# johannesschaeufele/CPUPathTrace

Measured on AMD Instinct MI355X. Metric: Msamples/s (all bounces), higher is better.
Workload: dtype f32

## Files before the change

### cpupathtrace_amd/csrc/pt_api.cpp

```cpp
#include "../../include/pt_hip.h"

#include <hip/hip_runtime.h>

#include <algorithm>
#include <chrono>
#include <cmath>
#include <cstdio>
#include <cstdlib>
#include <cstring>
#include <memory>
#include <mutex>
#include <string>
#include <thread>
#include <vector>

#include "pt_build.h"
#include "pt_bvh.h"
#include "pt_kernels.h"
#include "pt_post.h"

namespace {

thread_local std::string g_last_error;

// ... 102 lines not shown
struct pt_scene {
    int device = 0;
    hipStream_t stream = nullptr;
    int cu_count = 256;

    ptb::Tree tree;
    uint64_t n_nodes = 0;
    uint32_t depth = 0;
    bool device_built = false;
    float build_ms[4] = {0, 0, 0, 0};
    std::vector<uint32_t> tri_obj;
    std::vector<uint32_t> sph_obj;
    uint32_t n_objects = 0;
    uint32_t n_emissive = 0;
    std::vector<int32_t> emissive_obj;
    std::vector<float> emissive_cdf;

    DevBuf<F4> recs, pairs, tris, tri_shade, spheres, materials, lights, emis;
    DevBuf<uint2> sph_meta;
    DevBuf<float> emis_cdf;
    PtDevScene dev{};

    DevBuf<PtDevCounters> counters;
    DevBuf<F4> image;
    DevBuf<int4> tiles;
    DevBuf<uint32_t> tile_offset;
    DevBuf<float> batch_rays;

    std::mutex render_mutex;

    PtPathConfig path_cfg{};
    int path_blocks_per_cu = 0;
    uint32_t path_slots = 0, path_waves = 0, path_cap = 0;
    DevBuf<uint32_t> sl_stream, sl_nee_mask, pull_counter, tile_left;
    DevBuf<int4> sl_rect, st_rect;
    DevBuf<int32_t> sl_cursor, sl_path_length;
    DevBuf<uint64_t> sl_rng, st_rng;
    DevBuf<F4> sl_ray_o, sl_ray_d, sl_spectrum, sl_out, sl_nee, lq_ray_o, lq_ray_d;
    DevBuf<double> sl_divisor, sl_bounce_pd;
    DevBuf<PtEstimator> sl_est;
    DevBuf<PtCandidate> sl_cand;
    DevBuf<uint2> path_spill, closest_out;
    DevBuf<uint32_t> walk_save;
    DevBuf<PtPathArgs> path_args;
    PtPathArgs host_path_args{};
    DevBuf<unsigned long long> path_wave_counters;
    uint32_t *host_tiles_done = nullptr;
    unsigned long long *host_streams_done = nullptr;
    uint64_t streams_expected = 0;
    DevBuf<uint32_t> sl_cost, stream_cost, place;
    bool debug_collect_costs = false;
    std::vector<uint32_t> debug_place;
    uint32_t debug_place_waves = 0, debug_place_slots = 0;

    ~pt_scene() {
        if(host_tiles_done != nullptr) {
            (void)hipHostFree(host_tiles_done);
        }
        if(host_streams_done != nullptr) {
            (void)hipHostFree(host_streams_done);
        }
        if(stream != nullptr) {
            (void)hipStreamDestroy(stream);
        }
    }
};

namespace {

int device_count_quiet() {
    int n = 0;
    if(hipGetDeviceCount(&n) != hipSuccess) {
// ... 143 lines not shown
    if(slots_per_wave % first_lanes != 0) {
        if(slots_per_wave >= 64U) {
            slots_per_wave = (slots_per_wave + first_lanes - 1U) / first_lanes * first_lanes;
        }
        else {
            first_lanes = 1;
        }
    }
    cfg.first_lanes = static_cast<int>(first_lanes);
    int burst_default = 24;
    if(cfg.in_lds) {
        burst_default = slots_per_wave > 64U ? 12 : 24;
    }
    else if(slots_per_wave >= 64U) {
        burst_default = s->depth <= 12U ? 12 : (s->depth <= 18U ? 16 : 24);
    }
    cfg.burst_steps = std::min(std::max(env_int("PT_BURST", burst_default), 1), 64);
    int leaf_default = cfg.in_lds ? (slots_per_wave >= 64U ? 16 : 8) : static_cast<int>(std::min<uint32_t>(std::max<uint32_t>(slots_per_wave / 8U, 2U), 8U));
    if(!cfg.in_lds && slots_per_wave >= 64U && s->depth <= 24U) {
        leaf_default = 12;
    }
    cfg.leaf_min = std::min(std::max(env_int("PT_LEAF_MIN", leaf_default), 1), 64);
    const uint32_t rows = (slots_per_wave + 63U) / 64U;
    const uint32_t total = waves * rows * 64U;
    const uint32_t rays_per_slot = 1U + s->dev.n_lights + s->dev.n_object_samples;
    uint32_t cap = rows * 64U * rays_per_slot;
    const int ring_log = env_int("PT_RING_LOG_RAYS", 0);
    if(ring_log > 0) {
        cap = std::max<uint32_t>(cap, static_cast<uint32_t>(ring_log));
    }
    cfg.grid = static_cast<int>(grid);
    cfg.rows = static_cast<int>(rows);
    cfg.slots_per_wave = static_cast<int>(slots_per_wave);
    PT_HIP(s->sl_stream.ensure(total));
    PT_HIP(s->sl_rect.ensure(total));
    PT_HIP(s->sl_cursor.ensure(total));
    PT_HIP(s->sl_rng.ensure(total));
    PT_HIP(s->sl_ray_o.ensure(total));
    PT_HIP(s->sl_ray_d.ensure(total));
    PT_HIP(s->sl_spectrum.ensure(total));
    PT_HIP(s->sl_out.ensure(total));
    PT_HIP(s->sl_divisor.ensure(total));
    PT_HIP(s->sl_bounce_pd.ensure(total));
    PT_HIP(s->sl_path_length.ensure(total));
    PT_HIP(s->sl_nee.ensure(static_cast<size_t>(total) * std::max<uint32_t>(rays_per_slot - 1U, 1U)));
    PT_HIP(s->sl_nee_mask.ensure(total));
    PT_HIP(s->sl_cost.ensure(total));
    PT_HIP(s->sl_est.ensure(total));
    PT_HIP(s->sl_cand.ensure(static_cast<size_t>(total) * PT_MAX_CANDIDATES));
    PT_HIP(s->lq_ray_o.ensure(static_cast<size_t>(waves) * cap));
    PT_HIP(s->lq_ray_d.ensure(static_cast<size_t>(waves) * cap));
    if(ring_log > 0) {
        PT_HIP(hipMemsetAsync(s->lq_ray_d.ptr, 0xff, static_cast<size_t>(waves) * cap * 4 * sizeof(float), s->stream));
    }
    PT_HIP(s->path_spill.ensure(static_cast<size_t>(waves) * 64U * cfg.spill_depth));
    PT_HIP(s->path_wave_counters.ensure(static_cast<size_t>(waves) * 8U));
    PT_HIP(s->walk_save.ensure(static_cast<size_t>(waves) * 64U * PT_WALK_SAVE_WORDS));
    PT_HIP(s->pull_counter.ensure(64));
    PT_HIP(s->counters.ensure(1));
    cfg.spill = s->path_spill.ptr;
    cfg.walk_save = s->walk_save.ptr;
    cfg.wave_counters = s->path_wave_counters.ptr;
    s->path_slots = total;
    s->path_waves = waves;
    s->path_cap = cap;
    s->path_cfg.burst_steps = cfg.burst_steps;
    s->path_cfg.leaf_min = cfg.leaf_min;
    *out_cfg = cfg;
    return PT_OK;
}

int finish_path(pt_scene *s) {
    PT_HIP(hipStreamSynchronize(s->stream));
    if(s->host_streams_done != nullptr && s->streams_expected != 0) {
        const unsigned long long done = *static_cast<volatile unsigned long long *>(s->host_streams_done);
        const uint64_t expected = s->streams_expected;
        s->streams_expected = 0;
// ... 2 lines not shown
        }
    }
    return PT_OK;
}

int run_path(pt_scene *s, const PtDevCamera &cam, const PtDevOptions &opt, PtStreams T, float4 *d_image, pt_stats *stats, pt_progress_fn progress, void *progress_user,
             const PathPlan *plan = nullptr, bool want_costs = false) {
    PtPathConfig cfg;
    hipStream_t st = s->stream;
    PathPlan debug_plan;
    if(plan == nullptr && !s->debug_place.empty()) {
        PT_HIP(s->place.ensure(s->debug_place.size()));
        PT_HIP(hipMemcpyAsync(s->place.ptr, s->debug_place.data(), s->debug_place.size() * sizeof(uint32_t), hipMemcpyHostToDevice, st));
        PT_HIP(hipStreamSynchronize(st));
        debug_plan.waves = s->debug_place_waves;
        debug_plan.slots_per_wave = s->debug_place_slots;
        debug_plan.d_place = s->place.ptr;
        s->debug_place.clear();
        plan = &debug_plan;
    }
    int rc = ensure_path_workspace(s, T.n, &cfg, plan);
    if(rc != PT_OK) {
        return rc;
    }
    want_costs = want_costs || s->debug_collect_costs;
    T.place = plan != nullptr ? plan->d_place : nullptr;
    T.cost = nullptr;
    if(want_costs) {
        PT_HIP(s->stream_cost.ensure(std::max<uint32_t>(T.n, 1U)));
        T.cost = s->stream_cost.ptr;
    }
    PtSlots S{};
    S.total = s->path_slots;
    S.stream = s->sl_stream.ptr;
    S.rect = s->sl_rect.ptr;
    S.cursor = s->sl_cursor.ptr;
    S.rng = s->sl_rng.ptr;
    S.ray_o = reinterpret_cast<float4 *>(s->sl_ray_o.ptr);
    S.ray_d = reinterpret_cast<float4 *>(s->sl_ray_d.ptr);
    S.spectrum = reinterpret_cast<float4 *>(s->sl_spectrum.ptr);
    S.out = reinterpret_cast<float4 *>(s->sl_out.ptr);
    S.divisor = s->sl_divisor.ptr;
    S.bounce_pd = s->sl_bounce_pd.ptr;
    S.path_length = s->sl_path_length.ptr;
    S.nee = reinterpret_cast<float4 *>(s->sl_nee.ptr);
    S.nee_mask = s->sl_nee_mask.ptr;
    S.cost = s->sl_cost.ptr;
    S.est = s->sl_est.ptr;
    S.cand = s->sl_cand.ptr;
    PtLocalQueue Q{};
    Q.ray_o = reinterpret_cast<float4 *>(s->lq_ray_o.ptr);
    Q.ray_d = reinterpret_cast<float4 *>(s->lq_ray_d.ptr);
    Q.cap = s->path_cap;
    T.next = s->pull_counter.ptr;
    T.first_total = plan != nullptr ? T.n : s->path_waves * static_cast<uint32_t>(cfg.slots_per_wave);
    T.n_waves = s->path_waves;
    T.first_spread = env_int("PT_FIRST_SPREAD", 1) != 0 ? 1U : 0U;
    T.first_lanes = static_cast<uint32_t>(cfg.first_lanes);
    T.first_shift = static_cast<uint32_t>(std::max(env_int("PT_FIRST_SHIFT", 1), 0));
    {
        const uint32_t pieces = static_cast<uint32_t>(cfg.slots_per_wave) / T.first_lanes;
        const unsigned long long per_grid_row = static_cast<unsigned long long>(T.chunks_per_tile) * (64U / T.first_lanes) * T.tiles_per_row;
        if(env_int("PT_FIRST_SPREAD", 1) == 2 || per_grid_row == 0 || s->path_waves % per_grid_row != 0 || T.first_total > T.n || (T.tiles_per_row % pieces != 0 && pieces % T.tiles_per_row != 0)) {
            T.tiles_per_row = 0;
        }
    }
    T.tile_left = nullptr;
    T.tiles_done = nullptr;
    if(progress != nullptr && T.rect == nullptr && T.n_tiles > 0) {
        if(s->host_tiles_done == nullptr) {
            PT_HIP(hipHostMalloc(reinterpret_cast<void **>(&s->host_tiles_done), 64, hipHostMallocDefault));
        }
        *s->host_tiles_done = 0;
        T.tiles_done = s->host_tiles_done;
        T.tile_left = s->tile_left.ptr;
    }
    PT_HIP(hipMemsetAsync(s->counters.ptr, 0, sizeof(PtDevCounters), st));
// ... 1210 lines not shown
```

### cpupathtrace_amd/csrc/pt_kernels.h

```cpp
#ifndef PT_KERNELS_H
#define PT_KERNELS_H

#include <hip/hip_runtime.h>

#include "pt_types.h"

#define PT_F_DONE 1u
#define PT_F_IN_FLIGHT 2u
#define PT_F_HAS_EXT 4u
#define PT_F_COLLECTED 8u
#define PT_F_PIXEL 16u
#define PT_F_SAFE 64u
#define PT_F_OVERLAP 32u

#define PT_DEST_SHADOW 0x80000000u
#define PT_DEST_NULL 0xffffffffu


#define PT_LDS_TABLE_MAX 16
#define PT_LDS_TABLE_BYTES (PT_LDS_TABLE_MAX * (4 + 64 + 96 + 64))
#define PT_WALK_SAVE_WORDS 17
#define PT_MAX_ROWS 8
#define PT_F_STREAM 128u

struct PtSlots {
    uint32_t total;
    uint32_t *stream;
    int4 *rect;
    int32_t *cursor;
    uint64_t *rng;
    float4 *ray_o;
    float4 *ray_d;
    float4 *spectrum;
    float4 *out;
    double *divisor;
    double *bounce_pd;
    int32_t *path_length;
    float4 *nee;
    uint32_t *nee_mask;
    uint32_t *cost;
    PtEstimator *est;
    PtCandidate *cand;
};

struct PtStreams {
    uint32_t n;
    const int4 *rect;
    uint64_t *rng;
    const int4 *tiles;
    const uint32_t *tile_offset;
    uint32_t n_tiles;
    uint64_t base_seed;
    uint32_t first_total;
    uint32_t first_lanes;
    uint32_t first_shift;
    uint32_t n_waves, first_spread;
    uint32_t tiles_per_row, chunks_per_tile;
    uint32_t *next;
    uint32_t *tile_left;
    uint32_t *tiles_done;
    uint32_t *cost;
    const uint32_t *place;
};

struct PtLocalQueue {
    float4 *ray_o;
    float4 *ray_d;
    uint32_t cap;
};

// ... 54 lines not shown
```

### cpupathtrace_amd/csrc/pt_path.hip

```cpp
#include <type_traits>

#include "pt_device.h"
#include "pt_kernels.h"
#include "pt_shading.h"

using namespace ptd;

namespace {

typedef float f4v __attribute__((ext_vector_type(4)));
typedef float f2v __attribute__((ext_vector_type(2)));
typedef unsigned int u2v __attribute__((ext_vector_type(2)));
typedef const f4v __attribute__((address_space(3))) *lds_f4_cptr;
typedef const f4v __attribute__((address_space(1))) *glb_f4_cptr;
typedef u2v __attribute__((address_space(3))) *lds_u2_ptr;
typedef u2v __attribute__((address_space(1))) *glb_u2_ptr;
typedef unsigned int __attribute__((address_space(3))) *lds_u32_ptr;
typedef const PtPathArgs __attribute__((address_space(4))) *args_c4;

template<bool IN_LDS>
struct RecPtr {
    typedef glb_f4_cptr type;
};
template<>
// ... 73 lines not shown
#endif
    typedef typename RecPtr<IN_LDS>::type rec_ptr;
    rec_ptr recs;
    lds_u2_ptr stack_l;
    glb_u2_ptr my_spill;

    struct Rec {
        f4v r0, r1, r2, r3;
    };
    PT_D void fetch(uint32_t cur, Rec &R) const {
        rec_ptr p = recs + 4 * (size_t)(cur & PT_REF_INDEX);
        R.r0 = p[0];
        R.r1 = p[1];
        R.r2 = p[2];
        R.r3 = p[3];
    }
    static PT_D void whole(const Rec &R) {
        asm volatile("" ::"v"(R.r0), "v"(R.r1), "v"(R.r2), "v"(R.r3));
    }

    static PT_D unsigned long long node_lanes(uint32_t cur) { return __builtin_amdgcn_uicmp(cur, 0x40000000u, 36); }
    static PT_D unsigned long long slow_lanes(uint32_t cur) { return __builtin_amdgcn_uicmp(cur + 1u, 0x40000000u, 34); }

    PT_D void start(Walk &w, Rec &R, const RootBox &root, float4 ro, float4 rd) const {
        w.o = v3(ro.x, ro.y, ro.z);
        w.d = v3(rd.x, rd.y, rd.z);
        w.thr = ro.w;
        w.dest = __float_as_uint(rd.w);
        w.inv = slab_inverse(w.d);
        w.pack();
        w.best_ref = PT_REF_NONE;
        w.best_t = -1.0f;
        w.set_t_max(FLT_MAX);
        const u2v sentinel = {PT_REF_NONE, __float_as_uint(-1.0f)};
        stack_l[0] = sentinel;
        w.sp = 1;
        w.occluded = false;
        w.cur = PT_REF_NONE;
        if(root.ref != PT_REF_NONE) {
            const float t_root = slab_walk(ld3(root.lo), ld3(root.hi), w.o, w.inv);
            if(t_root >= 0.0f) {
                w.cur = root.ref;
                fetch(w.cur, R);
            }
        }
    }

    PT_D void node_step(Walk &w, Rec &R, unsigned long long node_mask, unsigned long long deep_mask) const {
        if(!__builtin_amdgcn_inverse_ballot_w64(node_mask)) {
            return;
        }
#ifdef PT_STEP_STAMPS
        asm volatile("s_waitcnt vmcnt(0)" ::: "memory");
#endif
        PT_STAMP(2);
        whole(R);
        const f4v q0 = R.r0, q1 = R.r1, q2 = R.r2;
        const uint32_t sp = w.sp;
        const u2v top = stack_l[((sp - 1u) & (uint32_t)(STACK_LDS - 1)) * 256u];
        const f2v a0 = ((f2v){q0.x, q0.y} - w.o_xy) * w.i_xy;
        const f2v a1 = ((f2v){q0.z, q0.w} - w.o_zx) * w.i_zx;
        const f2v a2 = ((f2v){q1.x, q1.y} - w.o_yz) * w.i_yz;
        const f2v a3 = ((f2v){q1.z, q1.w} - w.o_xy) * w.i_xy;
        const f2v a4 = ((f2v){q2.x, q2.y} - w.o_zx) * w.i_zx;
        const f2v a5 = ((f2v){q2.z, q2.w} - w.o_yz) * w.i_yz;
        const float l1 = a0.x, l2 = a1.y, l3 = a0.y, l4 = a2.x, l5 = a1.x, l6 = a2.y;
        const float r1 = a3.x, r2 = a4.y, r3 = a3.y, r4 = a5.x, r5 = a4.x, r6 = a5.y;
// ... 167 lines not shown
        if(T.tile_offset[mid] <= i) {
            lo = mid;
        }
        else {
            hi = mid;
        }
    }
    const int4 t = T.tiles[lo];
    const uint32_t k = i - T.tile_offset[lo];
    const int32_t x = t.x + (int32_t)(k % (uint32_t)t.z), y = t.y + (int32_t)(k / (uint32_t)t.z);
    rect = make_int4(x, y, 1, 1);
    const uint64_t seed = pixel_seed(T.base_seed, x, y);
    rng = seed ^ (~seed << 32);
    tile = lo;
}

struct EmisLds {
    const float __attribute__((address_space(3))) *cdf_l;
    lds_f4_cptr rec_l;
    lds_f4_cptr light_l;
    PT_D float cdf(int i) const { return cdf_l[i]; }
    PT_D float4 rec(int i, int k) const { return to_f4(rec_l[4 * i + k]); }
    PT_D V3 tri_normal_at(int i, uint32_t, V3 pos) const {
        uint32_t mat_unused;
        return tri_shade_normal(light_l + 6 * i, pos, mat_unused);
    }
};
struct ShadeTables {
    EmisLds emis;
    lds_f4_cptr materials_l;
    bool emis_in_lds, materials_in_lds;
};

template<bool WIDE>
PT_D void shade_row(const PtDevScene &sc, const PtDevCamera &cam, const PtDevOptions &opt, const PtSlots &S, const PtStreams &T, const PtLocalQueue &Q,
                    WaveCtx &ctx, uint32_t row, uint32_t ls_in, uint32_t lane, size_t slot_base, size_t queue_base, typename SlotWord<WIDE>::lds_ptr word_l, lds_u2_ptr hit_l,
                    float4 *__restrict__ image, PtDevCounters *counters, const ShadeTables &tb, uint32_t &n_samples, uint32_t &n_vertices) {
    const bool have_slot = ls_in != PT_NO_SLOT;
    const uint32_t ls = have_slot ? ls_in : 0u;
    const size_t p = slot_base + ls;
    const unsigned long long lt = (1ULL << lane) - 1ULL;
    const uint32_t n_light_samples = sc.n_lights + sc.n_object_samples;
    typedef SlotWord<WIDE> SW;
    const typename SW::T word = word_l[ls];
    uint32_t flags = SW::flags(word);
    const uint32_t vis_bits = SW::vis(word);
    bool ready = have_slot && !(flags & PT_F_DONE) && SW::pending(word) == 0;
    if(__ballot(ready) == 0ULL) {
        return;
    }

    {
        const bool want = ready && !(flags & PT_F_STREAM);
        const unsigned long long want_mask = __ballot(want);
        if(want_mask != 0ULL) {
            uint32_t base = T.n;
            uint32_t mine;
            if((ctx.first_rows >> row) & 1u) {
                ctx.first_rows &= ~(1u << row);
                base = ctx.first_base + row * 64u;
                mine = base + lane;
                if(T.place != nullptr) {
                    base = 0;
                    mine = T.place[ctx.first_base + ls];
                }
                else if(T.first_spread) {
                    const uint32_t g = T.first_lanes, q = row * (64u / g) + lane / g;
                    uint32_t chunk = q * T.n_waves + ctx.wave;
                    if(T.tiles_per_row != 0) {
                        const uint32_t per_tile = T.chunks_per_tile * (64u / g), pieces = (T.first_total / T.n_waves) / g;
                        const uint32_t tile = chunk / per_tile, sub = chunk % per_tile;
                        const uint32_t step = T.tiles_per_row >= pieces ? T.tiles_per_row / pieces : 1u;
                        const uint32_t tx = (tile % T.tiles_per_row + q * T.first_shift * step) % T.tiles_per_row, ty = tile / T.tiles_per_row;
                        chunk = (ty * T.tiles_per_row + tx) * per_tile + sub;
                    }
                    base = 0;
                    mine = chunk * g + lane % g;
                }
            }
            else {
                if(!ctx.pool_empty) {
                    if(lane == 0) {
                        base = T.first_total + atomicAdd(T.next, (uint32_t)__popcll(want_mask));
                    }
                    base = __builtin_amdgcn_readfirstlane(base);
                }
                mine = base + (uint32_t)__popcll(want_mask & lt);
                if(base >= T.n || base + (uint32_t)__popcll(want_mask) > T.n) {
                    ctx.pool_empty = true;
                }
            }
            const bool got = want && base < T.n && mine < T.n;
            if(got) {
                int4 rc;
                uint64_t r;
                uint32_t tile = 0;
                if(T.rect != nullptr) {
                    rc = T.rect[mine];
                    r = T.rng[mine];
                }
                else {
                    tile_stream(T, mine, rc, r, tile);
                }
                S.stream[p] = mine;
                S.rect[p] = rc;
                S.rng[p] = r;
                S.cursor[p] = 0;
                if(T.cost != nullptr) {
                    __hip_atomic_store(&S.cost[p], 0u, __ATOMIC_RELAXED, __HIP_MEMORY_SCOPE_AGENT);
                }
                flags = PT_F_STREAM;
            }
            else if(want) {
                flags = PT_F_DONE;
                ready = false;
                word_l[ls] = SW::make(PT_F_DONE, 0u, 0u, 0u);
            }
            ctx.n_dead += (uint32_t)__popcll(__ballot(want && !got));
        }
    }
    const bool alive = ready;
    uint32_t lane_samples = 0;

    uint64_t rng = 0;
    C4 out = c4(0, 0, 0, 0), spectrum = c4(1, 1, 1, 1);
    V3 ro = v3(0, 0, 0), rd = v3(0, 0, 1);
    float contribution_unweighted = 1.0f;
    double divisor = 1.0, bounce_pd = 1.0;
    int path_length = 0;
    bool shade_vertex = false;
    bool start_sample = false;
    float hit_t = -1.0f;
    uint32_t hit_ref = PT_REF_NONE;
    int4 rect = make_int4(0, 0, 0, 0);
    int32_t cursor = 0;
    bool stream_finished = false;

    if(alive) {
        rng = S.rng[p];
        rect = S.rect[p];
        cursor = S.cursor[p];
        if(flags & PT_F_IN_FLIGHT) {
            const float4 out4 = S.out[p];
            uint32_t mask = SW::waiting(word, S, p);
            const uint32_t lit = mask & vis_bits;
            float4 nee0 = make_float4(0, 0, 0, 0), nee1 = make_float4(0, 0, 0, 0);
            if(lit & 1u) {
                nee0 = S.nee[p];
            }
            if(lit & 2u) {
                nee1 = S.nee[S.total + p];
            }
            const float4 o4 = S.ray_o[p], d4 = S.ray_d[p], spectrum4 = S.spectrum[p];
            const double divisor_in = S.divisor[p], bounce_pd_in = S.bounce_pd[p];
            const int path_length_in = S.path_length[p];
            uint32_t warm = 0;
            if(flags & PT_F_HAS_EXT) {
                const u2v h = hit_l[ls];
                hit_t = __uint_as_float(h.x);
                hit_ref = h.y;
                if(!(hit_t < 0.0f) && !(hit_ref & PT_REF_SPHERE)) {
                    warm = *reinterpret_cast<const uint32_t *>(sc.tri_shade + 8 * (size_t)(hit_ref & PT_REF_INDEX));
                }
            }
            out = c4(out4);
            if(lit & 1u) {
                out = out + c4(nee0);
            }
            if(lit & 2u) {
                out = out + c4(nee1);
            }
            mask >>= 2;
            for(uint32_t j = 2; mask != 0; j++, mask >>= 1) {
                if((mask & 1u) && ((vis_bits >> j) & 1u)) {
                    out = out + c4(S.nee[(size_t)j * S.total + p]);
                }
            }
            asm volatile("" ::"v"(warm));
            if(flags & PT_F_OVERLAP) {
                PtEstimator e = S.est[p];
                out.a = 1.0f;
                (void)estimator_add(e, S.cand + p * PT_MAX_CANDIDATES, opt, out);
                e.pixel_sample++;
                lane_samples++;
                S.est[p] = e;
                flags &= ~(PT_F_OVERLAP | PT_F_COLLECTED | PT_F_SAFE);
                if(estimator_safe_to_overlap(e, opt)) {
                    flags |= PT_F_SAFE;
                }
                out = c4(0, 0, 0, 0);
            }
            bool finished = true;
            if((flags & PT_F_HAS_EXT) && !(hit_t < 0.0f)) {
                finished = false;
                shade_vertex = true;
            }
            if(finished) {
                PtEstimator e = S.est[p];
                PtCandidate *cand = S.cand + p * PT_MAX_CANDIDATES;
                bool accepted = false;
                if(flags & PT_F_COLLECTED) {
                    out.a = 1.0f;
                    accepted = estimator_add(e, cand, opt, out);
                }
                e.pixel_sample++;
                lane_samples++;
                if(accepted || e.pixel_sample >= opt.max_sample_count) {
                    const C4 value = estimator_finish(e, cand, opt, accepted);
                    const int32_t px = rect.x + cursor % rect.z, py = rect.y + cursor / rect.z;
                    image[(size_t)py * opt.image_width + px] = f4(value);
                    cursor++;
                    flags &= ~PT_F_PIXEL;
                }
                S.est[p] = e;
                flags &= ~(PT_F_IN_FLIGHT | PT_F_HAS_EXT | PT_F_COLLECTED | PT_F_SAFE);
                if((flags & PT_F_PIXEL) && estimator_safe_to_overlap(e, opt)) {
                    flags |= PT_F_SAFE;
                }
                start_sample = true;
            }
            else {
                ro = v3(o4.x, o4.y, o4.z);
                rd = v3(d4.x, d4.y, d4.z);
                contribution_unweighted = o4.w;
                spectrum = c4(spectrum4);
                divisor = divisor_in;
                bounce_pd = bounce_pd_in;
                path_length = path_length_in;
            }
        }
        else {
            start_sample = true;
        }
    }

    bool emit_ext = false;
    Ray ext;
    ext.o = v3(0, 0, 0);
    ext.d = v3(0, 0, 1);
    auto shoot_camera = [&](const int4 rc, int32_t cur) {
        const int32_t px = rc.x + cur % rc.z, py = rc.y + cur / rc.z;
        const float one_half = 1.0f / 2.0f;
        const float x_camera = 2 * (((float)px + one_half) / (float)opt.image_width - one_half);
        float y_camera = 2 * (((float)py + one_half) / (float)opt.image_height - one_half);
        y_camera = -y_camera;
        return camera_shoot(cam, x_camera, y_camera, opt.pixel_width, opt.pixel_height, rng);
    };
    if(start_sample) {
        bool have_pixel = false;
        while(cursor < rect.z * rect.w) {
            if(!(flags & PT_F_PIXEL)) {
                PtEstimator e;
                estimator_reset(e, opt);
                S.est[p] = e;
                flags = (flags | PT_F_PIXEL) & ~PT_F_SAFE;
                if(estimator_safe_to_overlap(e, opt)) {
                    flags |= PT_F_SAFE;
                }
                if(opt.max_sample_count <= 0) {
                    const int32_t px = rect.x + cursor % rect.z, py = rect.y + cursor / rect.z;
                    image[(size_t)py * opt.image_width + px] = make_float4(0.0f, 0.0f, 0.0f, 0.0f);
                    cursor++;
                    flags &= ~PT_F_PIXEL;
                    continue;
                }
            }
            have_pixel = true;
            break;
        }
        if(!have_pixel) {
            stream_finished = true;
            flags = 0;
        }
        else {
            ext = shoot_camera(rect, cursor);
            emit_ext = true;
            out = c4(0, 0, 0, 0);
            spectrum = c4(1, 1, 1, 1);
            contribution_unweighted = 1.0f;
            divisor = 1.0;
            bounce_pd = 1.0;
            path_length = 0;
            flags |= PT_F_IN_FLIGHT | PT_F_HAS_EXT;
        }
    }
    {
        const unsigned long long fin_mask = __ballot(stream_finished);
        if(fin_mask != 0ULL) {
            if(stream_finished) {
                const uint32_t si = S.stream[p];
                if(T.rng != nullptr) {
                    T.rng[si] = rng;
                }
                if(T.cost != nullptr) {
                    T.cost[si] = __hip_atomic_load(&S.cost[p], __ATOMIC_RELAXED, __HIP_MEMORY_SCOPE_AGENT);
                }
                if(T.tile_left != nullptr) {
                    int4 rc_unused;
                    uint64_t r_unused;
                    uint32_t tile = 0;
                    tile_stream(T, si, rc_unused, r_unused, tile);
                    if(atomicSub(&T.tile_left[tile], 1u) == 1u) {
                        __hip_atomic_fetch_add(T.tiles_done, 1u, __ATOMIC_RELAXED, __HIP_MEMORY_SCOPE_SYSTEM);
                    }
                }
            }
            if(lane == 0) {
                atomicAdd(&counters->streams_done, (unsigned long long)__popcll(fin_mask));
            }
        }
    }

    V3 pos = v3(0, 0, 0), n = v3(0, 1, 0);
    Material mat;
    mat.bsdf = 0;
    bool do_bounce = false;
    float bounce_probability = 1.0f;
    bool want_nee = false;
    bool safe_overlap = false;
    if(shade_vertex) {
        path_length++;
        flags |= PT_F_COLLECTED;
        pos = ro + rd * hit_t;
// ... 108 lines not shown
            }
        }
        const bool path_ends = !do_bounce || cancel_ext;
        if(path_ends && safe_overlap) {
            ext = shoot_camera(rect, cursor);
            spectrum = c4(1, 1, 1, 1);
            contribution_unweighted = 1.0f;
            divisor = 1.0;
            bounce_pd = 1.0;
            path_length = 0;
            flags |= PT_F_OVERLAP;
        }
        else if(path_ends && emit_ext) {
            Q.ray_d[ring(ext_pos)] = make_float4(0.0f, 0.0f, 0.0f, __uint_as_float(PT_DEST_NULL));
            emit_ext = false;
        }
        if(emit_ext) {
            flags |= PT_F_HAS_EXT;
        }
        else {
            flags &= ~PT_F_HAS_EXT;
        }
    }

    if(emit_ext) {
        const size_t at = ring(ext_pos);
        Q.ray_o[at] = make_float4(ext.o.x, ext.o.y, ext.o.z, 0.0f);
        Q.ray_d[at] = make_float4(ext.d.x, ext.d.y, ext.d.z, __uint_as_float(ls));
        n_rays++;
    }
    if(alive) {
        word_l[ls] = SW::make(flags, n_rays, vis_init, nee_out_mask);
        SW::keep_waiting(S, p, nee_out_mask);
        S.rng[p] = rng;
        S.cursor[p] = cursor;
        if(flags & PT_F_IN_FLIGHT) {
            S.ray_o[p] = make_float4(ext.o.x, ext.o.y, ext.o.z, contribution_unweighted);
            S.ray_d[p] = make_float4(ext.d.x, ext.d.y, ext.d.z, 0.0f);
            S.spectrum[p] = f4(spectrum);
            S.out[p] = f4(out);
            S.divisor[p] = divisor;
            S.bounce_pd[p] = bounce_pd;
            S.path_length[p] = path_length;
        }
    }
    n_samples += (uint32_t)__popcll(__ballot(lane_samples & 1u)) + 2u * (uint32_t)__popcll(__ballot((lane_samples & 2u) != 0u));
    n_vertices += (uint32_t)__popcll(__ballot(shade_vertex));
}


#define PT_PATH_STACK_LDS 8
#define PT_PATH_STACK_LDS_SMALL 4
#ifndef PT_COST_LDS_BYTES
#define PT_COST_LDS_BYTES 1024
#endif
#ifndef PT_PATH_WAVES
#define PT_PATH_WAVES 4
#endif

template<bool WIDE, bool IN_LDS, int STACK_LDS>
__global__ __launch_bounds__(256, PT_PATH_WAVES) void pt_path_kernel(const PtPathArgs *__restrict__ args) {
    typedef SlotWord<WIDE> SW;
    const args_c4 A4 = (args_c4)args;
    const PtPathArgs *A = (const PtPathArgs *)A4;
    const int rows = A->rows, slots_per_wave = A->slots_per_wave, refill_idle = A->refill_idle, min_ready = A->min_ready, burst_steps = A->burst_steps,
              leaf_min = A->leaf_min, ready_shift = A->ready_shift, pass_q_low = A->early_ready > 0 ? A->pass_q_low : 0, early_ready = A->early_ready;
    const unsigned long long lane_cap = A->debug_lanes >= 64 ? ~0ULL : ((1ULL << A->debug_lanes) - 1ULL);
    PtLocalQueue Q = A->Q;
    RootBox root;
    root.ref = A->sc.root_ref;
    for(int k = 0; k < 3; k++) {
        root.lo[k] = A->sc.root_lo[k];
        root.hi[k] = A->sc.root_hi[k];
    }
    extern __shared__ __align__(16) unsigned char lds_raw[];
    const int tid = threadIdx.x;
    const uint32_t lane = (uint32_t)tid & 63u;
    const uint32_t wave_in_block = __builtin_amdgcn_readfirstlane((uint32_t)tid >> 6);
    const uint32_t wave = blockIdx.x * 4u + wave_in_block;
    const uint32_t n_slots = (uint32_t)rows * 64u;
    unsigned char *at = lds_raw;
    lds_u2_ptr stack_l = (lds_u2_ptr)reinterpret_cast<uint2 *>(at) + tid;
    at += (size_t)STACK_LDS * 256 * sizeof(uint2);
    lds_u2_ptr hit_l = (lds_u2_ptr)reinterpret_cast<uint2 *>(at) + wave_in_block * n_slots;
    at += (size_t)4 * n_slots * sizeof(uint2);
    typename SW::lds_ptr word_l = (typename SW::lds_ptr)reinterpret_cast<typename SW::T *>(at) + wave_in_block * n_slots;
    at += (size_t)4 * n_slots * sizeof(typename SW::T);
    float *cdf_l = reinterpret_cast<float *>(at);
    at += (size_t)PT_LDS_TABLE_MAX * sizeof(float);
    float4 *emis_l = reinterpret_cast<float4 *>(at);
    at += (size_t)PT_LDS_TABLE_MAX * 4 * sizeof(float4);
    float4 *light_l = reinterpret_cast<float4 *>(at);
    at += (size_t)PT_LDS_TABLE_MAX * 6 * sizeof(float4);
    float4 *materials_l = reinterpret_cast<float4 *>(at);
    at += (size_t)PT_LDS_TABLE_MAX * 4 * sizeof(float4);
    uint32_t __attribute__((address_space(3))) *born_l = (uint32_t __attribute__((address_space(3))) *)reinterpret_cast<uint32_t *>(at) + tid;
    typedef unsigned char __attribute__((address_space(3))) *lds_u8_ptr;
    lds_u8_ptr list_l = (lds_u8_ptr)reinterpret_cast<unsigned char *>(at) + wave_in_block * 256u;
    at += (size_t)PT_COST_LDS_BYTES;
    float4 *lds_recs = reinterpret_cast<float4 *>(at);
    const bool cost_on = PT_COST_LDS_BYTES != 0 && A->T.cost != nullptr;
    uint32_t *const slot_cost = A->S.cost;

    ShadeTables tb;
    tb.emis.cdf_l = (const float __attribute__((address_space(3))) *)cdf_l;
    tb.emis.rec_l = (lds_f4_cptr)emis_l;
    tb.emis.light_l = (lds_f4_cptr)light_l;
    tb.materials_l = (lds_f4_cptr)materials_l;
    {
        const uint32_t n_emis = A->sc.n_emis, n_materials = A->sc.n_materials;
        tb.emis_in_lds = n_emis > 0 && n_emis <= PT_LDS_TABLE_MAX;
        tb.materials_in_lds = n_materials > 0 && n_materials <= PT_LDS_TABLE_MAX;
        if(tb.emis_in_lds) {
            const float4 *src_emis = A->sc.emis, *src_shade = A->sc.tri_shade;
            const float *src_cdf = A->sc.emis_cdf;
            for(uint32_t i = tid; i < n_emis; i += 256) {
                cdf_l[i] = src_cdf[i];
            }
            for(uint32_t i = tid; i < 4 * n_emis; i += 256) {
                emis_l[i] = src_emis[i];
            }
            for(uint32_t i = tid; i < 6 * n_emis; i += 256) {
                const uint32_t ref = __float_as_uint(src_emis[4 * (i / 6) + 2].y);
                light_l[i] = (ref & PT_REF_SPHERE) ? make_float4(0, 0, 0, 0) : src_shade[8 * (size_t)(ref & PT_REF_INDEX) + i % 6];
            }
        }
        if(tb.materials_in_lds) {
            const float4 *src_materials = A->sc.materials;
            for(uint32_t i = tid; i < 4 * n_materials; i += 256) {
                materials_l[i] = src_materials[i];
            }
        }
    }

    if(IN_LDS) {
        const uint32_t n_lds_quads = 4u * (A->sc.pair_base + A->sc.n_pairs);
        const float4 *src_recs = A->sc.recs;
        for(uint32_t i = tid; i < n_lds_quads; i += 256) {
            lds_recs[i] = src_recs[i];
        }
    }
    for(uint32_t i = lane; i < n_slots; i += 64) {
        word_l[i] = i < (uint32_t)slots_per_wave ? (typename SW::T)0 : SW::make(PT_F_DONE, 0u, 0u, 0u);
    }
    __syncthreads();

    Tracer<STACK_LDS, IN_LDS> tr;
    if(IN_LDS) {
        tr.recs = (typename RecPtr<IN_LDS>::type)(lds_f4_cptr)lds_recs;
    }
    else {
        tr.recs = (typename RecPtr<IN_LDS>::type)(glb_f4_cptr)A->sc.recs;
    }
    tr.stack_l = stack_l;
    tr.my_spill = (glb_u2_ptr)(A->spill + ((size_t)wave * 64 + lane) * A->spill_depth);

    const size_t slot_base = (size_t)wave * n_slots;
    const size_t queue_base = (size_t)wave * Q.cap;
    WaveCtx ctx;
    ctx.q_head = 0;
    ctx.q_count = 0;
    ctx.n_dead = n_slots - (uint32_t)slots_per_wave;
    ctx.pool_empty = false;
    ctx.first_rows = (1u << rows) - 1u;
    ctx.first_base = wave * (uint32_t)slots_per_wave;
    ctx.wave = wave;

    bool active = false;
    Walk w;
    w.o = v3(0, 0, 0);
    w.d = v3(0, 0, 1);
    w.inv = v3(0, 0, 0);
    w.pack();
    w.thr = 0.0f;
    w.dest = 0;
    w.best_t = 0.0f;
    w.best_ref = PT_REF_NONE;
    w.set_t_max(FLT_MAX);
    w.cur = PT_REF_NONE;
    w.sp = 0;
    w.occluded = false;
    typename Tracer<STACK_LDS, IN_LDS>::Rec rec;
    rec.r0 = rec.r1 = rec.r2 = rec.r3 = (f4v){0.0f, 0.0f, 0.0f, 0.0f};
    float4 win_o = make_float4(0, 0, 0, 0), win_d = make_float4(0, 0, 0, __uint_as_float(PT_DEST_NULL));
    uint32_t n_nodes = 0, n_leaves = 0, n_rays = 0, n_shadow = 0, n_samples = 0, n_vertices = 0;
    uint32_t w_steps = 0, w_passes = 0;
#ifdef PT_PATH_TIMING
    unsigned long long t_shade = 0, t_burst = 0;
    const unsigned long long t_begin = __builtin_amdgcn_s_memtime();
#endif

    bool want_pass = false;
    for(;;) {
        if(want_pass) {
            want_pass = false;
            w_passes++;
#ifdef PT_PATH_TIMING
            const unsigned long long t_pass = __builtin_amdgcn_s_memtime();
#endif
            size_t pass_offset = 0;
            asm volatile("" : "+s"(pass_offset));
            const PtPathArgs *P = (const PtPathArgs *)(args_c4)((const char __attribute__((address_space(4))) *)A4 + pass_offset);
            uint32_t *const walk_save = P->walk_save;
            const size_t save_stride = P->save_stride;
            {
                uint32_t *sv = walk_save + (size_t)wave * 64 + lane;
                const size_t st = save_stride;
                sv[0 * st] = __float_as_uint(w.o.x);
                sv[1 * st] = __float_as_uint(w.o.y);
                sv[2 * st] = __float_as_uint(w.o.z);
                sv[3 * st] = __float_as_uint(w.d.x);
                sv[4 * st] = __float_as_uint(w.d.y);
                sv[5 * st] = __float_as_uint(w.d.z);
                sv[6 * st] = __float_as_uint(w.thr);
                sv[7 * st] = w.dest;
                sv[8 * st] = __float_as_uint(w.best_t);
                sv[9 * st] = w.best_ref;
                sv[10 * st] = __float_as_uint(w.t_max);
                sv[11 * st] = w.cur;
                sv[12 * st] = w.sp | (w.occluded ? 0x80000000u : 0u);
                sv[13 * st] = n_nodes;
                sv[14 * st] = n_leaves;
                sv[15 * st] = n_rays;
                sv[16 * st] = n_shadow;
            }
            uint32_t n_listed = 0;
            bool compact = false;
            if(PT_COST_LDS_BYTES >= 1024 && !cost_on && P->compact_passes != 0 && rows > 1 && rows <= 4 && ctx.first_rows == 0u) {
                uint32_t rows_used = 0;
                for(uint32_t r = 0; r < (uint32_t)rows; r++) {
                    const typename SW::T word = word_l[r * 64 + lane];
                    const bool is_ready = !(SW::flags(word) & PT_F_DONE) && SW::pending(word) == 0;
                    const unsigned long long m = __ballot(is_ready);
                    if(is_ready) {
                        list_l[n_listed + (uint32_t)__popcll(m & ((1ULL << lane) - 1ULL))] = (unsigned char)(r * 64 + lane);
                    }
                    n_listed += (uint32_t)__popcll(m);
                    rows_used += m != 0ULL ? 1u : 0u;
                }
                compact = (n_listed + 63u) / 64u < rows_used;
                __builtin_amdgcn_fence(__ATOMIC_ACQ_REL, "workgroup");
            }
            const uint32_t n_chunks = compact ? (n_listed + 63u) / 64u : (uint32_t)rows;
#pragma unroll 1
            for(uint32_t k = 0; k < n_chunks; k++) {
                uint32_t ls = k * 64u + lane;
                if(compact) {
                    ls = ls < n_listed ? (uint32_t)list_l[ls] : PT_NO_SLOT;
                }
                shade_row<WIDE>(P->sc, P->cam, P->opt, P->S, P->T, P->Q, ctx, k, ls, lane, slot_base, queue_base, word_l, hit_l, P->image, P->counters, tb, n_samples, n_vertices);
            }
            __builtin_amdgcn_fence(__ATOMIC_ACQ_REL, "workgroup");
            __builtin_amdgcn_s_waitcnt(0);
            {
                asm volatile("" : "+s"(pass_offset));
                const PtPathArgs *R = (const PtPathArgs *)(args_c4)((const char __attribute__((address_space(4))) *)A4 + pass_offset);
                const uint32_t *sv = R->walk_save + (size_t)wave * 64 + lane;
                const size_t st = R->save_stride;
                w.o = v3(__uint_as_float(sv[0 * st]), __uint_as_float(sv[1 * st]), __uint_as_float(sv[2 * st]));
                w.d = v3(__uint_as_float(sv[3 * st]), __uint_as_float(sv[4 * st]), __uint_as_float(sv[5 * st]));
                w.inv = slab_inverse(w.d);
                w.pack();
                w.thr = __uint_as_float(sv[6 * st]);
                w.dest = sv[7 * st];
                w.best_t = __uint_as_float(sv[8 * st]);
                w.best_ref = sv[9 * st];
                w.set_t_max(__uint_as_float(sv[10 * st]));
                w.cur = sv[11 * st];
                const uint32_t packed = sv[12 * st];
                w.sp = packed & 0x7fffffffu;
                w.occluded = (packed >> 31) != 0;
                n_nodes = sv[13 * st];
                n_leaves = sv[14 * st];
                n_rays = sv[15 * st];
                n_shadow = sv[16 * st];
            }
#ifdef PT_PATH_TIMING
            t_shade += __builtin_amdgcn_s_memtime() - t_pass;
#endif
            win_o = make_float4(0, 0, 0, 0);
            win_d = make_float4(0, 0, 0, __uint_as_float(PT_DEST_NULL));
            if(lane < ctx.q_count) {
                uint32_t i = ctx.q_head + lane;
                i = i >= Q.cap ? i - Q.cap : i;
                win_o = Q.ray_o[queue_base + i];
                win_d = Q.ray_d[queue_base + i];
            }
            rec.r0 = rec.r1 = rec.r2 = rec.r3 = (f4v){0.0f, 0.0f, 0.0f, 0.0f};
                    if(active && w.cur < PT_REF_POPPING) {
                tr.fetch(w.cur, rec);
            }
        }

        bool finished = false;
        for(;;) {
            if(active && w.cur == PT_REF_NONE) {
                const uint32_t ls = w.dest & PT_DEST_SLOT_MASK;
                if(w.dest & PT_DEST_SHADOW) {
                    const uint32_t j = (w.dest >> PT_DEST_J_SHIFT) & SW::j_mask;
                    __hip_atomic_fetch_add(&word_l[ls], (typename SW::T)(w.occluded ? 0u : (1u << j)) - SW::one_ray(), __ATOMIC_RELAXED, __HIP_MEMORY_SCOPE_WORKGROUP);
                }
                else {
                    const u2v h = {__float_as_uint(w.best_ref == PT_REF_NONE ? -1.0f : w.best_t), w.best_ref};
                    hit_l[ls] = h;
                    __hip_atomic_fetch_add(&word_l[ls], (typename SW::T)0 - SW::one_ray(), __ATOMIC_RELAXED, __HIP_MEMORY_SCOPE_WORKGROUP);
                }
                if(cost_on) {
                    __hip_atomic_fetch_add(&slot_cost[slot_base + ls], w_steps - *born_l, __ATOMIC_RELAXED, __HIP_MEMORY_SCOPE_AGENT);
                }
                active = false;
            }

            const unsigned long long idle_mask = __ballot(!active) & lane_cap;
            const uint32_t n_idle = (uint32_t)__popcll(idle_mask);
            if(n_idle >= (uint32_t)refill_idle) {
                if(ctx.q_count <= (uint32_t)pass_q_low && ctx.n_dead < n_slots) {
                    uint32_t n_ready = 0;
                    for(uint32_t r = 0; r < (uint32_t)rows; r++) {
                        const typename SW::T word = word_l[r * 64 + lane];
                        n_ready += (uint32_t)__popcll(__ballot(!(SW::flags(word) & PT_F_DONE) && SW::pending(word) == 0));
                    }
                    const uint32_t live_share = (n_slots - ctx.n_dead) >> ready_shift;
                    const uint32_t need = live_share < (uint32_t)min_ready ? (live_share > 1u ? live_share : 1u) : (uint32_t)min_ready;
                    if(ctx.q_count == 0 ? (n_ready >= need || n_idle == (uint32_t)__popcll(lane_cap)) : n_ready >= (uint32_t)early_ready) {
                        want_pass = true;
                        break;
                    }
                }
                if(ctx.q_count > 0) {
                    const uint32_t take = ctx.q_count < n_idle ? ctx.q_count : n_idle;
                    const uint32_t rank = (uint32_t)__popcll(idle_mask & ((1ULL << lane) - 1ULL));
                    const int src = (int)(rank & 63u);
                    const float4 ro = make_float4(__shfl(win_o.x, src), __shfl(win_o.y, src), __shfl(win_o.z, src), __shfl(win_o.w, src));
                    const float4 rd = make_float4(__shfl(win_d.x, src), __shfl(win_d.y, src), __shfl(win_d.z, src), __shfl(win_d.w, src));
                    if(!active && rank < take && __float_as_uint(rd.w) != PT_DEST_NULL) {
                        tr.start(w, rec, root, ro, rd);
                        if(cost_on) {
                            *born_l = w_steps;
                        }
                        active = true;
                        n_rays++;
                        n_shadow += (w.dest & PT_DEST_SHADOW) ? 1u : 0u;
                    }
                    ctx.q_head += take;
                    ctx.q_head = ctx.q_head >= Q.cap ? ctx.q_head - Q.cap : ctx.q_head;
                    ctx.q_count -= take;
                    if(lane < ctx.q_count) {
                        uint32_t i = ctx.q_head + lane;
                        i = i >= Q.cap ? i - Q.cap : i;
                        win_o = Q.ray_o[queue_base + i];
                        win_d = Q.ray_d[queue_base + i];
                    }
                }
            }
            if(__ballot(active) == 0ULL) {
                if(ctx.q_count == 0 && ctx.n_dead >= n_slots) {
                    finished = true;
                    break;
                }
                continue;
            }

#ifdef PT_PATH_TIMING
            const unsigned long long t_b0 = __builtin_amdgcn_s_memtime();
#endif
#pragma unroll 1
            for(int burst = 0; burst < burst_steps; burst++) {
// ... 386 lines not shown
```

Baseline: 452.1.

## Pack per-slot path state into one planar buffer and rematerialize lane IDs

Replaces eleven separate per-slot arrays (stream, rect, cursor, rng, rays, spectrum, out, divisor, bounce_pd, path_length) with a single plane-indexed float4 state buffer. Related fields are packed into 16-byte vectors (rng+cursor+stream, divisor+bounce_pd, path_length in ray_d.w), so each access is one wide load or store with 32-bit indexing. The kernel also recomputes the lane index with mbcnt, swaps __shfl for ds_bpermute, and moves in asm sentinel constants, all to cut register pressure across the shading pass. It adds a 4 GiB limit check on the slot state and relies on inline asm tricks that depend on the compiler.

```diff
diff --git a/cpupathtrace_amd/csrc/pt_api.cpp b/cpupathtrace_amd/csrc/pt_api.cpp
--- a/cpupathtrace_amd/csrc/pt_api.cpp
+++ b/cpupathtrace_amd/csrc/pt_api.cpp
@@ -158,12 +158,10 @@
     PtPathConfig path_cfg{};
     int path_blocks_per_cu = 0;
     uint32_t path_slots = 0, path_waves = 0, path_cap = 0;
-    DevBuf<uint32_t> sl_stream, sl_nee_mask, pull_counter, tile_left;
-    DevBuf<int4> sl_rect, st_rect;
-    DevBuf<int32_t> sl_cursor, sl_path_length;
-    DevBuf<uint64_t> sl_rng, st_rng;
-    DevBuf<F4> sl_ray_o, sl_ray_d, sl_spectrum, sl_out, sl_nee, lq_ray_o, lq_ray_d;
-    DevBuf<double> sl_divisor, sl_bounce_pd;
+    DevBuf<uint32_t> sl_nee_mask, pull_counter, tile_left;
+    DevBuf<int4> st_rect;
+    DevBuf<uint64_t> st_rng;
+    DevBuf<F4> sl_state, sl_nee, lq_ray_o, lq_ray_d;
     DevBuf<PtEstimator> sl_est;
     DevBuf<PtCandidate> sl_cand;
     DevBuf<uint2> path_spill, closest_out;
@@ -373,17 +371,10 @@
     cfg.grid = static_cast<int>(grid);
     cfg.rows = static_cast<int>(rows);
     cfg.slots_per_wave = static_cast<int>(slots_per_wave);
-    PT_HIP(s->sl_stream.ensure(total));
-    PT_HIP(s->sl_rect.ensure(total));
-    PT_HIP(s->sl_cursor.ensure(total));
-    PT_HIP(s->sl_rng.ensure(total));
-    PT_HIP(s->sl_ray_o.ensure(total));
-    PT_HIP(s->sl_ray_d.ensure(total));
-    PT_HIP(s->sl_spectrum.ensure(total));
-    PT_HIP(s->sl_out.ensure(total));
-    PT_HIP(s->sl_divisor.ensure(total));
-    PT_HIP(s->sl_bounce_pd.ensure(total));
-    PT_HIP(s->sl_path_length.ensure(total));
+    if(static_cast<unsigned long long>(total) * PT_SLOT_PLANES * sizeof(F4) > 0xffffffffULL) {
+        return fail(PT_ERR_UNSUPPORTED, "path kernel: " + std::to_string(total) + " slots do not fit the 4 GiB the slot state may occupy");
+    }
+    PT_HIP(s->sl_state.ensure(static_cast<size_t>(total) * PT_SLOT_PLANES));
     PT_HIP(s->sl_nee.ensure(static_cast<size_t>(total) * std::max<uint32_t>(rays_per_slot - 1U, 1U)));
     PT_HIP(s->sl_nee_mask.ensure(total));
     PT_HIP(s->sl_cost.ensure(total));
@@ -452,17 +443,7 @@
     }
     PtSlots S{};
     S.total = s->path_slots;
-    S.stream = s->sl_stream.ptr;
-    S.rect = s->sl_rect.ptr;
-    S.cursor = s->sl_cursor.ptr;
-    S.rng = s->sl_rng.ptr;
-    S.ray_o = reinterpret_cast<float4 *>(s->sl_ray_o.ptr);
-    S.ray_d = reinterpret_cast<float4 *>(s->sl_ray_d.ptr);
-    S.spectrum = reinterpret_cast<float4 *>(s->sl_spectrum.ptr);
-    S.out = reinterpret_cast<float4 *>(s->sl_out.ptr);
-    S.divisor = s->sl_divisor.ptr;
-    S.bounce_pd = s->sl_bounce_pd.ptr;
-    S.path_length = s->sl_path_length.ptr;
+    S.state = reinterpret_cast<float4 *>(s->sl_state.ptr);
     S.nee = reinterpret_cast<float4 *>(s->sl_nee.ptr);
     S.nee_mask = s->sl_nee_mask.ptr;
     S.cost = s->sl_cost.ptr;
diff --git a/cpupathtrace_amd/csrc/pt_kernels.h b/cpupathtrace_amd/csrc/pt_kernels.h
--- a/cpupathtrace_amd/csrc/pt_kernels.h
+++ b/cpupathtrace_amd/csrc/pt_kernels.h
@@ -23,19 +23,17 @@
 #define PT_MAX_ROWS 8
 #define PT_F_STREAM 128u
 
+#define PT_PLANE_RAY_O 0
+#define PT_PLANE_RAY_D 1
+#define PT_PLANE_PD 2
+#define PT_PLANE_ENGINE 3
+#define PT_PLANE_SPECTRUM 4
+#define PT_PLANE_OUT 5
+#define PT_PLANE_RECT 6
+#define PT_SLOT_PLANES 7
 struct PtSlots {
     uint32_t total;
-    uint32_t *stream;
-    int4 *rect;
-    int32_t *cursor;
-    uint64_t *rng;
-    float4 *ray_o;
-    float4 *ray_d;
-    float4 *spectrum;
-    float4 *out;
-    double *divisor;
-    double *bounce_pd;
-    int32_t *path_length;
+    float4 *state;
     float4 *nee;
     uint32_t *nee_mask;
     uint32_t *cost;
diff --git a/cpupathtrace_amd/csrc/pt_path.hip b/cpupathtrace_amd/csrc/pt_path.hip
--- a/cpupathtrace_amd/csrc/pt_path.hip
+++ b/cpupathtrace_amd/csrc/pt_path.hip
@@ -129,7 +129,9 @@
         w.best_ref = PT_REF_NONE;
         w.best_t = -1.0f;
         w.set_t_max(FLT_MAX);
-        const u2v sentinel = {PT_REF_NONE, __float_as_uint(-1.0f)};
+        uint32_t sent_ref, sent_t;
+        asm volatile("v_mov_b32 %0, -1\n\tv_mov_b32 %1, -1.0" : "=v"(sent_ref), "=v"(sent_t));
+        const u2v sentinel = {sent_ref, sent_t};
         stack_l[0] = sentinel;
         w.sp = 1;
         w.occluded = false;
@@ -363,13 +365,18 @@
     bool emis_in_lds, materials_in_lds;
 };
 
+template<typename V>
+PT_D V *slot_plane(const PtSlots &S, uint32_t k, uint32_t p) {
+    return reinterpret_cast<V *>(reinterpret_cast<char *>(S.state) + (k * S.total + p) * (uint32_t)sizeof(float4));
+}
+
 template<bool WIDE>
 PT_D void shade_row(const PtDevScene &sc, const PtDevCamera &cam, const PtDevOptions &opt, const PtSlots &S, const PtStreams &T, const PtLocalQueue &Q,
-                    WaveCtx &ctx, uint32_t row, uint32_t ls_in, uint32_t lane, size_t slot_base, size_t queue_base, typename SlotWord<WIDE>::lds_ptr word_l, lds_u2_ptr hit_l,
+                    WaveCtx &ctx, uint32_t row, uint32_t ls_in, uint32_t lane, uint32_t slot_base, size_t queue_base, typename SlotWord<WIDE>::lds_ptr word_l, lds_u2_ptr hit_l,
                     float4 *__restrict__ image, PtDevCounters *counters, const ShadeTables &tb, uint32_t &n_samples, uint32_t &n_vertices) {
     const bool have_slot = ls_in != PT_NO_SLOT;
     const uint32_t ls = have_slot ? ls_in : 0u;
-    const size_t p = slot_base + ls;
+    const uint32_t p = slot_base + ls;
     const unsigned long long lt = (1ULL << lane) - 1ULL;
     const uint32_t n_light_samples = sc.n_lights + sc.n_object_samples;
     typedef SlotWord<WIDE> SW;
@@ -433,10 +440,8 @@
                 else {
                     tile_stream(T, mine, rc, r, tile);
                 }
-                S.stream[p] = mine;
-                S.rect[p] = rc;
-                S.rng[p] = r;
-                S.cursor[p] = 0;
+                *slot_plane<int4>(S, PT_PLANE_RECT, p) = rc;
+                *slot_plane<uint4>(S, PT_PLANE_ENGINE, p) = make_uint4((uint32_t)r, (uint32_t)(r >> 32), 0u, mine);
                 if(T.cost != nullptr) {
                     __hip_atomic_store(&S.cost[p], 0u, __ATOMIC_RELAXED, __HIP_MEMORY_SCOPE_AGENT);
                 }
@@ -465,14 +470,17 @@
     uint32_t hit_ref = PT_REF_NONE;
     int4 rect = make_int4(0, 0, 0, 0);
     int32_t cursor = 0;
+    uint32_t stream = 0;
     bool stream_finished = false;
 
     if(alive) {
-        rng = S.rng[p];
-        rect = S.rect[p];
-        cursor = S.cursor[p];
+        const uint4 engine = *slot_plane<uint4>(S, PT_PLANE_ENGINE, p);
+        rng = (uint64_t)engine.x | ((uint64_t)engine.y << 32);
+        cursor = (int32_t)engine.z;
+        stream = engine.w;
+        rect = *slot_plane<int4>(S, PT_PLANE_RECT, p);
         if(flags & PT_F_IN_FLIGHT) {
-            const float4 out4 = S.out[p];
+            const float4 out4 = *slot_plane<float4>(S, PT_PLANE_OUT, p);
             uint32_t mask = SW::waiting(word, S, p);
             const uint32_t lit = mask & vis_bits;
             float4 nee0 = make_float4(0, 0, 0, 0), nee1 = make_float4(0, 0, 0, 0);
@@ -482,9 +490,9 @@
             if(lit & 2u) {
                 nee1 = S.nee[S.total + p];
             }
-            const float4 o4 = S.ray_o[p], d4 = S.ray_d[p], spectrum4 = S.spectrum[p];
-            const double divisor_in = S.divisor[p], bounce_pd_in = S.bounce_pd[p];
-            const int path_length_in = S.path_length[p];
+            const float4 o4 = *slot_plane<float4>(S, PT_PLANE_RAY_O, p), d4 = *slot_plane<float4>(S, PT_PLANE_RAY_D, p);
+            const float4 spectrum4 = *slot_plane<float4>(S, PT_PLANE_SPECTRUM, p);
+            const double2 pd_in = *slot_plane<double2>(S, PT_PLANE_PD, p);
             uint32_t warm = 0;
             if(flags & PT_F_HAS_EXT) {
                 const u2v h = hit_l[ls];
@@ -511,7 +519,7 @@
             if(flags & PT_F_OVERLAP) {
                 PtEstimator e = S.est[p];
                 out.a = 1.0f;
-                (void)estimator_add(e, S.cand + p * PT_MAX_CANDIDATES, opt, out);
+                (void)estimator_add(e, S.cand + (size_t)p * PT_MAX_CANDIDATES, opt, out);
                 e.pixel_sample++;
                 lane_samples++;
                 S.est[p] = e;
@@ -528,7 +536,7 @@
             }
             if(finished) {
                 PtEstimator e = S.est[p];
-                PtCandidate *cand = S.cand + p * PT_MAX_CANDIDATES;
+                PtCandidate *cand = S.cand + (size_t)p * PT_MAX_CANDIDATES;
                 bool accepted = false;
                 if(flags & PT_F_COLLECTED) {
                     out.a = 1.0f;
@@ -555,9 +563,9 @@
                 rd = v3(d4.x, d4.y, d4.z);
                 contribution_unweighted = o4.w;
                 spectrum = c4(spectrum4);
-                divisor = divisor_in;
-                bounce_pd = bounce_pd_in;
-                path_length = path_length_in;
+                divisor = pd_in.x;
+                bounce_pd = pd_in.y;
+                path_length = __float_as_int(d4.w);
             }
         }
         else {
@@ -619,7 +627,7 @@
         const unsigned long long fin_mask = __ballot(stream_finished);
         if(fin_mask != 0ULL) {
             if(stream_finished) {
-                const uint32_t si = S.stream[p];
+                const uint32_t si = stream;
                 if(T.rng != nullptr) {
                     T.rng[si] = rng;
                 }
@@ -794,16 +802,13 @@
     if(alive) {
         word_l[ls] = SW::make(flags, n_rays, vis_init, nee_out_mask);
         SW::keep_waiting(S, p, nee_out_mask);
-        S.rng[p] = rng;
-        S.cursor[p] = cursor;
+        *slot_plane<uint3>(S, PT_PLANE_ENGINE, p) = make_uint3((uint32_t)rng, (uint32_t)(rng >> 32), (uint32_t)cursor);
         if(flags & PT_F_IN_FLIGHT) {
-            S.ray_o[p] = make_float4(ext.o.x, ext.o.y, ext.o.z, contribution_unweighted);
-            S.ray_d[p] = make_float4(ext.d.x, ext.d.y, ext.d.z, 0.0f);
-            S.spectrum[p] = f4(spectrum);
-            S.out[p] = f4(out);
-            S.divisor[p] = divisor;
-            S.bounce_pd[p] = bounce_pd;
-            S.path_length[p] = path_length;
+            *slot_plane<float4>(S, PT_PLANE_RAY_O, p) = make_float4(ext.o.x, ext.o.y, ext.o.z, contribution_unweighted);
+            *slot_plane<float4>(S, PT_PLANE_RAY_D, p) = make_float4(ext.d.x, ext.d.y, ext.d.z, __int_as_float(path_length));
+            *slot_plane<float4>(S, PT_PLANE_SPECTRUM, p) = f4(spectrum);
+            *slot_plane<float4>(S, PT_PLANE_OUT, p) = f4(out);
+            *slot_plane<double2>(S, PT_PLANE_PD, p) = make_double2(divisor, bounce_pd);
         }
     }
     n_samples += (uint32_t)__popcll(__ballot(lane_samples & 1u)) + 2u * (uint32_t)__popcll(__ballot((lane_samples & 2u) != 0u));
@@ -819,6 +824,12 @@
 #ifndef PT_PATH_WAVES
 #define PT_PATH_WAVES 4
 #endif
+
+PT_D uint32_t lane_afresh() {
+    uint32_t l;
+    asm volatile("v_mbcnt_lo_u32_b32 %0, -1, 0\n\tv_mbcnt_hi_u32_b32 %0, -1, %0" : "=v"(l));
+    return l;
+}
 
 template<bool WIDE, bool IN_LDS, int STACK_LDS>
 __global__ __launch_bounds__(256, PT_PATH_WAVES) void pt_path_kernel(const PtPathArgs *__restrict__ args) {
@@ -837,12 +848,12 @@
     }
     extern __shared__ __align__(16) unsigned char lds_raw[];
     const int tid = threadIdx.x;
-    const uint32_t lane = (uint32_t)tid & 63u;
+    uint32_t lane = (uint32_t)tid & 63u;
     const uint32_t wave_in_block = __builtin_amdgcn_readfirstlane((uint32_t)tid >> 6);
     const uint32_t wave = blockIdx.x * 4u + wave_in_block;
     const uint32_t n_slots = (uint32_t)rows * 64u;
     unsigned char *at = lds_raw;
-    lds_u2_ptr stack_l = (lds_u2_ptr)reinterpret_cast<uint2 *>(at) + tid;
+    const lds_u2_ptr stack_base = (lds_u2_ptr)reinterpret_cast<uint2 *>(at) + wave_in_block * 64u;
     at += (size_t)STACK_LDS * 256 * sizeof(uint2);
     lds_u2_ptr hit_l = (lds_u2_ptr)reinterpret_cast<uint2 *>(at) + wave_in_block * n_slots;
     at += (size_t)4 * n_slots * sizeof(uint2);
@@ -856,7 +867,9 @@
     at += (size_t)PT_LDS_TABLE_MAX * 6 * sizeof(float4);
     float4 *materials_l = reinterpret_cast<float4 *>(at);
     at += (size_t)PT_LDS_TABLE_MAX * 4 * sizeof(float4);
-    uint32_t __attribute__((address_space(3))) *born_l = (uint32_t __attribute__((address_space(3))) *)reinterpret_cast<uint32_t *>(at) + tid;
+    typedef uint32_t __attribute__((address_space(3))) *lds_u32_ptr;
+    const lds_u32_ptr born_base = (lds_u32_ptr)reinterpret_cast<uint32_t *>(at) + wave_in_block * 64u;
+    lds_u32_ptr born_l = born_base + lane;
     typedef unsigned char __attribute__((address_space(3))) *lds_u8_ptr;
     lds_u8_ptr list_l = (lds_u8_ptr)reinterpret_cast<unsigned char *>(at) + wave_in_block * 256u;
     at += (size_t)PT_COST_LDS_BYTES;
@@ -914,8 +927,12 @@
     else {
         tr.recs = (typename RecPtr<IN_LDS>::type)(glb_f4_cptr)A->sc.recs;
     }
-    tr.stack_l = stack_l;
-    tr.my_spill = (glb_u2_ptr)(A->spill + ((size_t)wave * 64 + lane) * A->spill_depth);
+    auto bind_lane = [&](const PtPathArgs *B, uint32_t l) {
+        lane = l;
+        tr.stack_l = stack_base + l;
+        tr.my_spill = (glb_u2_ptr)(B->spill + ((size_t)wave * 64 + l) * B->spill_depth);
+        born_l = born_base + l;
+    };
 
     const size_t slot_base = (size_t)wave * n_slots;
     const size_t queue_base = (size_t)wave * Q.cap;
@@ -965,8 +982,9 @@
             const PtPathArgs *P = (const PtPathArgs *)(args_c4)((const char __attribute__((address_space(4))) *)A4 + pass_offset);
             uint32_t *const walk_save = P->walk_save;
             const size_t save_stride = P->save_stride;
+            const uint32_t lane_s = lane_afresh();
             {
-                uint32_t *sv = walk_save + (size_t)wave * 64 + lane;
+                uint32_t *sv = walk_save + (size_t)wave * 64 + lane_s;
                 const size_t st = save_stride;
                 sv[0 * st] = __float_as_uint(w.o.x);
                 sv[1 * st] = __float_as_uint(w.o.y);
@@ -991,11 +1009,11 @@
             if(PT_COST_LDS_BYTES >= 1024 && !cost_on && P->compact_passes != 0 && rows > 1 && rows <= 4 && ctx.first_rows == 0u) {
                 uint32_t rows_used = 0;
                 for(uint32_t r = 0; r < (uint32_t)rows; r++) {
-                    const typename SW::T word = word_l[r * 64 + lane];
+                    const typename SW::T word = word_l[r * 64 + lane_s];
                     const bool is_ready = !(SW::flags(word) & PT_F_DONE) && SW::pending(word) == 0;
                     const unsigned long long m = __ballot(is_ready);
                     if(is_ready) {
-                        list_l[n_listed + (uint32_t)__popcll(m & ((1ULL << lane) - 1ULL))] = (unsigned char)(r * 64 + lane);
+                        list_l[n_listed + (uint32_t)__popcll(m & ((1ULL << lane_s) - 1ULL))] = (unsigned char)(r * 64 + lane_s);
                     }
                     n_listed += (uint32_t)__popcll(m);
                     rows_used += m != 0ULL ? 1u : 0u;
@@ -1006,18 +1024,18 @@
             const uint32_t n_chunks = compact ? (n_listed + 63u) / 64u : (uint32_t)rows;
 #pragma unroll 1
             for(uint32_t k = 0; k < n_chunks; k++) {
-                uint32_t ls = k * 64u + lane;
+                uint32_t ls = k * 64u + lane_s;
                 if(compact) {
                     ls = ls < n_listed ? (uint32_t)list_l[ls] : PT_NO_SLOT;
                 }
-                shade_row<WIDE>(P->sc, P->cam, P->opt, P->S, P->T, P->Q, ctx, k, ls, lane, slot_base, queue_base, word_l, hit_l, P->image, P->counters, tb, n_samples, n_vertices);
+                shade_row<WIDE>(P->sc, P->cam, P->opt, P->S, P->T, P->Q, ctx, k, ls, lane_s, (uint32_t)slot_base, queue_base, word_l, hit_l, P->image, P->counters, tb, n_samples, n_vertices);
             }
             __builtin_amdgcn_fence(__ATOMIC_ACQ_REL, "workgroup");
             __builtin_amdgcn_s_waitcnt(0);
             {
                 asm volatile("" : "+s"(pass_offset));
                 const PtPathArgs *R = (const PtPathArgs *)(args_c4)((const char __attribute__((address_space(4))) *)A4 + pass_offset);
-                const uint32_t *sv = R->walk_save + (size_t)wave * 64 + lane;
+                const uint32_t *sv = R->walk_save + (size_t)wave * 64 + lane_afresh();
                 const size_t st = R->save_stride;
                 w.o = v3(__uint_as_float(sv[0 * st]), __uint_as_float(sv[1 * st]), __uint_as_float(sv[2 * st]));
                 w.d = v3(__uint_as_float(sv[3 * st]), __uint_as_float(sv[4 * st]), __uint_as_float(sv[5 * st]));
@@ -1042,8 +1060,9 @@
 #endif
             win_o = make_float4(0, 0, 0, 0);
             win_d = make_float4(0, 0, 0, __uint_as_float(PT_DEST_NULL));
-            if(lane < ctx.q_count) {
-                uint32_t i = ctx.q_head + lane;
+            const uint32_t lane_w = lane_afresh();
+            if(lane_w < ctx.q_count) {
+                uint32_t i = ctx.q_head + lane_w;
                 i = i >= Q.cap ? i - Q.cap : i;
                 win_o = Q.ray_o[queue_base + i];
                 win_d = Q.ray_d[queue_base + i];
@@ -1054,6 +1073,11 @@
             }
         }
 
+        {
+            size_t bind_offset = 0;
+            asm volatile("" : "+s"(bind_offset));
+            bind_lane((const PtPathArgs *)(args_c4)((const char __attribute__((address_space(4))) *)A4 + bind_offset), lane_afresh());
+        }
         bool finished = false;
         for(;;) {
             if(active && w.cur == PT_REF_NONE) {
@@ -1093,8 +1117,9 @@
                     const uint32_t take = ctx.q_count < n_idle ? ctx.q_count : n_idle;
                     const uint32_t rank = (uint32_t)__popcll(idle_mask & ((1ULL << lane) - 1ULL));
                     const int src = (int)(rank & 63u);
-                    const float4 ro = make_float4(__shfl(win_o.x, src), __shfl(win_o.y, src), __shfl(win_o.z, src), __shfl(win_o.w, src));
-                    const float4 rd = make_float4(__shfl(win_d.x, src), __shfl(win_d.y, src), __shfl(win_d.z, src), __shfl(win_d.w, src));
+                    auto from = [src](float v) { return __int_as_float(__builtin_amdgcn_ds_bpermute(src << 2, __float_as_int(v))); };
+                    const float4 ro = make_float4(from(win_o.x), from(win_o.y), from(win_o.z), from(win_o.w));
+                    const float4 rd = make_float4(from(win_d.x), from(win_d.y), from(win_d.z), from(win_d.w));
                     if(!active && rank < take && __float_as_uint(rd.w) != PT_DEST_NULL) {
                         tr.start(w, rec, root, ro, rd);
                         if(cost_on) {
```

After: 469.3 (median of 6 runs). 1.04x the previous value.
